# openstack/pyeclib

Measured on AMD Instinct MI355X. Metric: device-resident encode+decode GiB/s, k=10 m=4, 4 MiB objects, 1/2/4/8 GPU, higher is better.
Workload: dtype u16

## Files before the change

### pyeclib_amd/csrc/ec_kernels_impl.hpp

```cpp
#pragma once

#include <algorithm>
#include <cstdlib>
#include <cstddef>
#include <type_traits>
#include <atomic>
#include <map>
#include <mutex>
#include <tuple>
#include <utility>
#include <unordered_map>

#include "crc32.hpp"
#include "crc_device.hpp"
#include "ec_crc.hpp"
#include "ec_kernels.hpp"

namespace ecamd {
namespace {

typedef __attribute__((address_space(3))) char lds_char;
typedef unsigned int v2u __attribute__((ext_vector_type(2)));
typedef unsigned int v4u __attribute__((ext_vector_type(4)));
__device__ __forceinline__ uint2 lds_u64(uint32_t a, uint32_t tab) {
  const v2u v = *reinterpret_cast<const __attribute__((address_space(3))) v2u*>(
      reinterpret_cast<const lds_char*>(static_cast<uintptr_t>(a)) + tab);
  return make_uint2(v.x, v.y);
}
__device__ __forceinline__ uint32_t lds_u32(uint32_t a, uint32_t tab) {
  return *reinterpret_cast<const __attribute__((address_space(3))) uint32_t*>(
      reinterpret_cast<const lds_char*>(static_cast<uintptr_t>(a)) + tab);
}
__device__ __forceinline__ __attribute__((address_space(3))) v4u* lds_v4(uint32_t byte) {
  return reinterpret_cast<__attribute__((address_space(3))) v4u*>(static_cast<uintptr_t>(byte));
}

__device__ __forceinline__ uint4 ld_stream(const void* p) {
  const v4u v = __builtin_nontemporal_load(reinterpret_cast<const v4u*>(p));
  return make_uint4(v.x, v.y, v.z, v.w);
}
__device__ __forceinline__ void st_stream(void* p, const uint4& x) {
  v4u v;
  v.x = x.x;
  v.y = x.y;
  v.z = x.z;
  v.w = x.w;
  __builtin_nontemporal_store(v, reinterpret_cast<v4u*>(p));
}

typedef __amdgpu_buffer_rsrc_t Rsrc;
constexpr int kNt = 2;
__device__ __forceinline__ uint32_t to_sgpr(uint32_t v);
__device__ __forceinline__ Rsrc rsrc(const void* base, int records = -1) {
  const uint64_t a = reinterpret_cast<uint64_t>(base);
  const uint32_t lo = __builtin_amdgcn_readfirstlane(static_cast<uint32_t>(a));
  const uint32_t hi = __builtin_amdgcn_readfirstlane(static_cast<uint32_t>(a >> 32));
  const int n = static_cast<int>(to_sgpr(static_cast<uint32_t>(records)));
  return __builtin_amdgcn_make_buffer_rsrc(
      reinterpret_cast<void*>((static_cast<uint64_t>(hi) << 32) | lo), 0, n, 0x00020000);
}
template <bool CACHED = false>
__device__ __forceinline__ uint4 buf_ld(Rsrc r, uint32_t voff, uint32_t soff) {
  const v4u v = __builtin_amdgcn_raw_buffer_load_b128(r, voff, soff, CACHED ? 0 : kNt);
  return make_uint4(v.x, v.y, v.z, v.w);
}
__device__ __forceinline__ void st_fence() {
  __builtin_amdgcn_sched_barrier(0);
  asm volatile("s_nop 0");
  __builtin_amdgcn_sched_barrier(0);
}

template <bool CACHED = false>
__device__ __forceinline__ void buf_st(Rsrc r, uint32_t voff, uint32_t soff, const uint4& x) {
  v4u v;
  v.x = x.x;
  v.y = x.y;
  v.z = x.z;
  v.w = x.w;
  __builtin_amdgcn_raw_buffer_store_b128(v, r, voff, soff, CACHED ? 0 : kNt);
  st_fence();
}

__device__ __forceinline__ void lookup_fence() {
  __builtin_amdgcn_sched_barrier(0);
  asm volatile("" ::: "memory");
}

__device__ __forceinline__ uint32_t xor3(uint32_t a, uint32_t b, uint32_t c) {
  return __builtin_amdgcn_bitop3_b32(a, b, c, 0x96);
}


#define ECAMD_SDWA_AND_BYTE(B)                                                              \
  "v_and_b32_sdwa %0, %1, %2 dst_sel:DWORD dst_unused:UNUSED_PAD src0_sel:BYTE_" #B \
  " src1_sel:DWORD"
template <int B>
__device__ __forceinline__ uint32_t hi_nib16(uint32_t x) {
// ... 580 lines not shown
__host__ __device__ constexpr int encode_occ() {
  if (F::kRows > kRowsPerPass) return 4;
  if (CRC) return DATA ? kEncodeCrcDataOcc : (stream_bufs<K>() >= 6 ? 6 : kEncodeCrcOcc);
  if (DATA) return kEncodeDataOcc;
  if (NBX > 6) return 4;
  if (F::kW == 8 && K >= 18) return 7;
  return kEncodeOcc;
}

template <class F, int K, int NR, bool NOCOMP = false, bool DATA = false, int CH = 1,
          bool NTL = false, int NBX = 0, bool HEAD = false, bool CRC = false>
__global__ void __launch_bounds__(kThreadsPerBlock)
    __attribute__((amdgpu_waves_per_eu(encode_occ<F, K, DATA, NBX, CRC>(), 8)))
    encode_kernel(EncodeParams p) {
  load_tables(p.tables, K * F::kTableBytes, 0);
  if constexpr (CRC)
    load_tables(static_cast<const uint32_t*>(p.crc_lanes), kCrcLaneBytes, crc_lds_base<F, K>());
  __syncthreads();
  if (p.fused_edges) {
    if (p.edge_blocks == 0) {
      encode_edges<F, K, NR, DATA>(p, gridDim.x - 1 - blockIdx.x, gridDim.x);
    } else if (blockIdx.x < p.edge_blocks) {
      encode_edges<F, K, NR, DATA>(p, blockIdx.x, p.edge_blocks);
      return;
    }
  }
  encode_interior<F, K, NR, NOCOMP, DATA, CH, NTL, NBX, HEAD, CRC>(p);
}

template <class F, int K, int NR>
__global__ void __launch_bounds__(kThreadsPerBlock) encode_edge_kernel(EncodeParams p) {
  load_tables(p.tables, K * F::kTableBytes, 0);
  __syncthreads();
  encode_edges<F, K, NR, false>(p, blockIdx.x, gridDim.x);
}

constexpr uint32_t kDmaSlot = 8192;
constexpr uint32_t kDmaThreads = 512;

typedef unsigned int v4u_s __attribute__((ext_vector_type(4)));
__device__ __forceinline__ v4u_s rsrc4(const void* base, uint32_t records) {
  const uint64_t a = reinterpret_cast<uint64_t>(base);
  v4u_s r;
  r.x = __builtin_amdgcn_readfirstlane(static_cast<uint32_t>(a));
  r.y = __builtin_amdgcn_readfirstlane(static_cast<uint32_t>(a >> 32)) & 0xFFFFu;
  r.z = to_sgpr(records);
  r.w = 0x00020000u;
  return r;
}
template <bool NT>
__device__ __forceinline__ void dma16(v4u_s r, uint32_t voff, uint32_t soff, uint32_t lds) {
  uint32_t keep;
  if constexpr (NT)
    asm volatile(
        "s_mov_b32 %0, m0\n\ts_mov_b32 m0, %3\n\ts_nop 0\n\t"
        "buffer_load_dwordx4 %1, %2, %4 offen nt lds\n\ts_mov_b32 m0, %0"
        : "=&s"(keep) : "v"(voff), "s"(r), "s"(lds), "s"(soff) : "memory");
  else
    asm volatile(
        "s_mov_b32 %0, m0\n\ts_mov_b32 m0, %3\n\ts_nop 0\n\t"
        "buffer_load_dwordx4 %1, %2, %4 offen lds\n\ts_mov_b32 m0, %0"
        : "=&s"(keep) : "v"(voff), "s"(r), "s"(lds), "s"(soff) : "memory");
}
template <int N>
__device__ __forceinline__ void wait_vm() {
  static_assert(N >= 0 && N <= 63, "vmcnt range");
  asm volatile("s_waitcnt vmcnt(%0)" ::"n"(N) : "memory");
}
__device__ __forceinline__ void ring_barrier() {
  asm volatile("s_waitcnt lgkmcnt(0)" ::: "memory");
  __builtin_amdgcn_s_barrier();
  asm volatile("" ::: "memory");
}

template <class F, int K>
__host__ __device__ constexpr uint32_t dma_ring_base() {
  return (K * F::kTableBytes + 255u) & ~255u;
}
template <class F, int K, int R, int SW, int W = 8>
__host__ __device__ constexpr uint32_t dma_lds_bytes(bool crc = false) {
  return dma_ring_base<F, K>() + (crc ? kCrcLaneBytes : 0u) + R * 1024 * W * SW;
}

template <class F, int K, int NR, int R, bool NT, int L = 4, int SW = 1, int W = 8,
          bool DATA = false, bool NOCOMP = false, bool CONTIG = false, int RUNS = 0, int COMB = 0,
          int CV = 6>
__global__ void __launch_bounds__(W * 64) encode_dma_kernel(EncodeParams p) {
  static_assert(R >= 2 && R <= K + 1, "ring of 2 .. K + 1 slots");
  static_assert(L == 2 || L == 4 || L == 8 || L == 16, "loader waves");
  constexpr uint32_t kSlot = 1024u * W * SW;
  constexpr int kPerLoader = kSlot / 1024 / L;
  const uint32_t wave = wave_in_block();
  if (blockIdx.x < p.edge_blocks) {
    if (threadIdx.x >= kThreadsPerBlock) return;
    for (uint32_t i = threadIdx.x; i < K * F::kTableBytes / 16; i += kThreadsPerBlock)
      lds_v4(0)[i] = reinterpret_cast<const v4u*>(p.tables)[i];
    __syncthreads();
    encode_edges<F, K, NR, DATA>(p, blockIdx.x, p.edge_blocks);
    return;
  }
  const bool crc = p.crc_lanes != nullptr;
  for (uint32_t i = threadIdx.x; i < K * F::kTableBytes / 16; i += W * 64)
    lds_v4(0)[i] = reinterpret_cast<const v4u*>(p.tables)[i];
  if (crc)
    load_tables(static_cast<const uint32_t*>(p.crc_lanes), kCrcLaneBytes, dma_ring_base<F, K>(), W * 64);
  __syncthreads();
  ItemRange rg = item_range(p.n_obj * p.tiles, p.xcd_split, interior_block(p.edge_blocks));
  if constexpr (CONTIG) {
    const uint64_t nall = static_cast<uint64_t>(p.n_obj) * p.tiles;
    const IBlock ib = interior_block(p.edge_blocks);
    rg = {static_cast<uint32_t>(__builtin_amdgcn_readfirstlane(static_cast<uint32_t>(nall * ib.b / ib.g))),
          static_cast<uint32_t>(__builtin_amdgcn_readfirstlane(static_cast<uint32_t>(nall * (ib.b + 1) / ib.g))),
          1u};
  }
  uint32_t n_items = 0;
  const IBlock ibk = interior_block(p.edge_blocks);
  const uint32_t nall = p.n_obj * p.tiles;
  const uint32_t runs_total = RUNS ? (nall + RUNS - 1) / RUNS : 0;
  const uint32_t groups = COMB ? ibk.g / COMB : 1, r0 = COMB ? ibk.b % COMB : 0;
  const uint32_t per_obj = COMB ? (p.tiles > r0 ? (p.tiles - r0 + COMB - 1) / COMB : 0) : 0;
  if constexpr (COMB > 0) {
    const uint32_t g0 = ibk.b / COMB;
    if (per_obj == 0 || g0 >= p.n_obj || ibk.b >= groups * COMB) return;
    n_items = to_sgpr((p.n_obj - g0 + groups - 1) / groups * per_obj);
  } else if constexpr (RUNS > 0) {
    if (ibk.b >= runs_total) return;
    n_items = (runs_total - ibk.b + ibk.g - 1) / ibk.g * RUNS;
    if ((runs_total - 1 - ibk.b) % ibk.g == 0) n_items -= runs_total * RUNS - nall;
    n_items = to_sgpr(n_items);
  } else {
    if (rg.begin >= rg.end) return;
    n_items = to_sgpr((rg.end - rg.begin + rg.step - 1) / rg.step);
  }
  const bool loader = wave < static_cast<uint32_t>(L);
  const uint32_t lane16 = lane_id() * 16, lane4 = lane_id() * 4;
  const uint32_t kRing = to_sgpr(dma_ring_base<F, K>() + (crc ? kCrcLaneBytes : 0u));
  const uint32_t chunks = crc_chunks(p.tiles, p.tile_ch);
  auto item_at = [&](uint32_t i, uint32_t& o, uint32_t& x0) {
    if constexpr (COMB > 0) {
      const uint32_t q = i / per_obj, sidx = i - q * per_obj;
      o = to_sgpr(ibk.b / COMB + q * groups);
      x0 = (r0 + sidx * COMB) * kSlot;
      return;
    }
    const uint32_t w = RUNS ? (ibk.b + ibk.g * (i / (RUNS ? RUNS : 1))) * RUNS + i % (RUNS ? RUNS : 1)
                            : rg.begin + i * rg.step;
    o = to_sgpr(w / p.tiles);
    x0 = (w - o * p.tiles) * kSlot;
  };
  auto issue = [&](uint32_t i, int j, uint32_t ri) {
    if (!loader) return;
    uint32_t o, x0;
    const bool valid = i < n_items;
    item_at(valid ? i : 0, o, x0);
    const v4u_s src = rsrc4(p.objs + static_cast<uint64_t>(o) * p.obj_stride, valid ? ~0u : 0u);
    const uint32_t part = wave * (kSlot / L);
    const uint32_t lds = kRing + ri * kSlot + part;
    const uint32_t soff = to_sgpr(j * p.bs + x0 + part);
#pragma unroll
    for (int c = 0; c < kPerLoader; ++c) dma16<NT>(src, lane16, soff + 1024 * c, lds + 1024 * c);
  };
#pragma unroll
  for (int t = 0; t < R - 1; ++t) issue(t / K, t % K, t);
  uint32_t ring = 0;
  typename F::Acc s[SW];
#pragma unroll
  for (int c = 0; c < SW; ++c) F::zero(s[c]);
  constexpr bool kMf = CV == 4 || CV == 6;
  constexpr bool kMf4 = CV == 6;
  constexpr int kPerRow = kMf ? 9 : 5;
  constexpr int kCrcSteps = kPerRow * NR + (kMf4 ? 1 : 0);
  static_assert(!kMf4 || NR <= 4, "one joint wave XOR");
  uint32_t cfin[kMf4 ? 4 : 1] = {};
  uint4 crow[NR];
  uint32_t cacc[NR];
  uint32_t* cpart = p.crc_part;
  bool cpend = false;
  crcdev::mfma_v4i mb[kMf ? 8 : 1];
  crcdev::mfma_v16i macc = {};
  if constexpr (kMf) {
    if (crc) crcdev::mfma_load_b(p.crc_lanes, lane_id(), mb);
  }
  uint32_t dfin[kMf4 && DATA ? 4 : 1] = {};
  uint4 xprev = {};
  uint32_t* dprev = nullptr;
  bool dpend = false;
  auto data_crc = [&](int c, uint32_t* base) {
    if constexpr (kMf4 && DATA) {
      crcdev::mfma_v16i dacc = {};
#pragma unroll
      for (int d = 0; d < 8; ++d) dacc = crcdev::mfma_plane(xprev, d, mb[d], d == 0 ? crcdev::mfma_v16i{} : dacc);
      dfin[c % 4] = crcdev::mfma_lanes(dacc, dma_ring_base<F, K>() + offsetof(CrcLaneTables, mst), lane4);
      if (c % 4 == 3 || c == K - 1) {
        const int n = c % 4 + 1;
        const uint32_t t = crcdev::wave_xor4(dfin[0], n > 1 ? dfin[1] : 0u, n > 2 ? dfin[2] : 0u,
                                             n > 3 ? dfin[3] : 0u, lane_id());
        if (lane_id() < static_cast<uint32_t>(n)) base[c + 1 - n + lane_id()] = t;
      }
    }
  };
  auto crc_step = [&](int u) {
    if constexpr (kMf4) {
      if (u == kPerRow * NR) {
        const uint32_t t = crcdev::wave_xor4(cfin[0], cfin[1], cfin[2], cfin[3], lane_id());
        if (lane_id() < p.nrows && lane_id() < static_cast<uint32_t>(NR)) cpart[lane_id()] = t;
        return;
      }
      const int q = u / kPerRow, d = u % kPerRow;
      if (d < 8)
        macc = crcdev::mfma_plane(crow[q], d, mb[d], d == 0 ? crcdev::mfma_v16i{} : macc);
      else
        cfin[q] = crcdev::mfma_lanes(macc, dma_ring_base<F, K>() + offsetof(CrcLaneTables, mst), lane4);
      return;
    }
    if constexpr (kMf) {
      const int q = u / kPerRow, d = u % kPerRow;
      if (d < 8) {
        macc = crcdev::mfma_plane(crow[q], d, mb[d], d == 0 ? crcdev::mfma_v16i{} : macc);
      } else if (static_cast<uint32_t>(q) < p.nrows) {
        crc_store(cpart + q, crcdev::mfma_finish(macc, dma_ring_base<F, K>() + offsetof(CrcLaneTables, mst), lane4));
      }
      return;
    }
    const int q = u / kPerRow, d = u % kPerRow;
    if (d < 4) {
      const uint32_t w = d == 0 ? crow[q].x : d == 1 ? crow[q].y : d == 2 ? crow[q].z : crow[q].w;
      cacc[q] ^= crcdev::raw_dword(w, d, dma_ring_base<F, K>());
    } else if (static_cast<uint32_t>(q) < p.nrows) {
      crc_store(cpart + q, crcdev::wave_xor(crcdev::lane_map(
                               cacc[q], dma_ring_base<F, K>() + offsetof(CrcLaneTables, lane), lane4)));
    }
  };
#pragma clang loop unroll(disable)
  for (uint32_t i = 0; i < n_items; ++i) {
    uint32_t o, x0;
    item_at(i, o, x0);
    const Rsrc par = rsrc_parity(p, o);
    Rsrc dat;
    if constexpr (DATA) dat = rsrc_data(p, o);
#pragma unroll
    for (int j = 0; j < K; ++j) {
      if (loader) wait_vm<kPerLoader * (R - 2)>();
      ring_barrier();
      const uint32_t rn = ring == 0 ? R - 1 : ring - 1;
      issue(i + (j + R - 1) / K, (j + R - 1) % K, rn);
#pragma unroll
      for (int c = 0; c < SW; ++c) {
        const v4u xin = *lds_v4(kRing + ring * kSlot + (wave * SW + c) * 1024 + lane16);
        const uint4 x = make_uint4(xin.x, xin.y, xin.z, xin.w);
        if constexpr (NOCOMP) {
          uint32_t* a = reinterpret_cast<uint32_t*>(&s[c]);
          a[0] ^= x.x;
        } else {
          F::template mac<true>(F::kb(0), j * F::kTableBytes, x, s[c]);
        }
        if constexpr (DATA) {
          buf_st(dat, lane16, j * p.frag_stride + kHeaderBytes + x0 + (wave * SW + c) * 1024, x);
          uint32_t* dpart = p.crc_part_data + (static_cast<uint64_t>(o) * chunks + x0 / 1024 + wave * SW + c) * K;
          if constexpr (kMf4 && SW == 1) {
            if (crc) {
              if (j > 0) data_crc(j - 1, dpart);
              else if (dpend) data_crc(K - 1, dprev);
              xprev = x;
              if (j == K - 1) {
                dprev = dpart;
                dpend = true;
              }
            }
          } else if (crc) {
            crc_store(dpart + j, crcdev::chunk_crc(x, dma_ring_base<F, K>(), lane4));
          }
        }
      }
      if constexpr (SW == 1 && (CV == 0 || CV == 4 || CV == 6)) {
        if (cpend) {
#pragma unroll
          for (int u = j * kCrcSteps / K; u < (j + 1) * kCrcSteps / K; ++u) crc_step(u);
        }
      }
      ring = ring + 1 == R ? 0 : ring + 1;
    }
#pragma unroll
    for (int c = 0; c < SW; ++c) {
      F::pin(s[c]);
      const uint32_t soff = p.row0 * p.frag_stride + kHeaderBytes + x0 + (wave * SW + c) * 1024;
#pragma unroll
      for (int q = 0; q < NR; ++q)
        buf_st(parity_row<NR>(p, o, q, par), lane16, soff + q * p.frag_stride, F::row(s[c], q));
      if (crc) {
        uint32_t* part = p.crc_part + (static_cast<uint64_t>(o) * chunks + x0 / 1024 + wave * SW + c) * p.m + p.row0;
        if constexpr (SW == 1 && (CV == 0 || CV == 4 || CV == 6)) {
#pragma unroll
          for (int q = 0; q < NR; ++q) {
            crow[q] = F::row(s[c], q);
            cacc[q] = 0;
          }
          cpart = part;
          cpend = true;
        } else {
#pragma unroll
          for (int q = 0; q < NR; ++q)
            if (static_cast<uint32_t>(q) < p.nrows)
              crc_store(part + q, crcdev::chunk_crc<CV == 2>(F::row(s[c], q), dma_ring_base<F, K>(), lane4));
        }
      }
      F::zero(s[c]);
    }
  }
  if constexpr (kMf4 && DATA && SW == 1) {
    if (crc && dpend) data_crc(K - 1, dprev);
  }
  if constexpr (SW == 1 && (CV == 0 || CV == 4 || CV == 6)) {
    if (cpend) {
#pragma unroll
      for (int u = 0; u < kCrcSteps; ++u) crc_step(u);
    }
  }
  if (loader) wait_vm<0>();
}

__global__ void __launch_bounds__(kThreadsPerBlock) __attribute__((unused))
    copy_data_kernel(EncodeParams p) {
  const uint32_t per_frag = (p.bs + kTile - 1) / kTile;
  const uint32_t per_obj = p.k * per_frag;
  const uint32_t items = p.n_obj * per_obj;
  for (uint32_t w = blockIdx.x; w < items; w += gridDim.x) {
    const uint32_t o = w / per_obj, rest = w - o * per_obj;
    const uint32_t j = rest / per_frag, c = rest - j * per_frag;
    const uint32_t t = c * kTile + threadIdx.x * 16;
    if (t >= p.bs) continue;
    const uint8_t* obj = p.objs + static_cast<uint64_t>(o) * p.obj_stride;
    const uint4 x = load_clamped(obj, static_cast<uint64_t>(j) * p.bs + t, p.obj_len);
    store_partial(p.data + static_cast<uint64_t>(o) * p.stripe_stride + j * p.frag_stride +
                      kHeaderBytes + t,
                  x, static_cast<int64_t>(p.bs) - t);
  }
}


struct Slots {
  uint32_t table;
  uint32_t slot;
};

template <class F, int K>
struct TablePre {
  static constexpr int kChunks = K * F::kTableBytes / 16;
  static constexpr int kPer = (kChunks + kThreadsPerBlock - 1) / kThreadsPerBlock;
  uint4 v[kPer];
  uint32_t table;
};

template <class F, int K>
__device__ __forceinline__ void table_prefetch(const DecodeParams& p, uint32_t table, bool need,
                                               TablePre<F, K>& pre) {
  constexpr uint32_t kBytes = K * F::kTableBytes;
  const Rsrc t = rsrc(p.tables + static_cast<uint64_t>(table) * (kBytes / 4), need ? kBytes : 0);
#pragma unroll
  for (int i = 0; i < TablePre<F, K>::kPer; ++i)
    pre.v[i] = buf_ld<true>(t, (threadIdx.x + i * kThreadsPerBlock) * 16, 0);
  pre.table = need ? table : 0xFFFFFFFFu;
}

template <class F, int K, class D>
__device__ __forceinline__ uint32_t ensure_tables(const DecodeParams& p, const D& d, Slots& st,
                                                  const TablePre<F, K>& pre) {
  constexpr uint32_t kSlot = table_slot_bytes(K, F::kW);
  if (d.n_out() != 0 && d.table() != st.table) {
    st.slot ^= 1u;
    const uint32_t base = st.slot * kSlot;
    if (pre.table == d.table()) {
      auto* dst = lds_v4(base);
#pragma unroll
      for (int i = 0; i < TablePre<F, K>::kPer; ++i) {
        const uint32_t c = threadIdx.x + i * kThreadsPerBlock;
        if (c < static_cast<uint32_t>(TablePre<F, K>::kChunks)) {
          v4u v;
          v.x = pre.v[i].x;
          v.y = pre.v[i].y;
          v.z = pre.v[i].z;
          v.w = pre.v[i].w;
          dst[c] = v;
        }
      }
    } else {
      load_tables(p.tables + static_cast<uint64_t>(d.table()) * (K * F::kTableBytes / 4),
                  K * F::kTableBytes, base, kThreadsPerBlock);
    }
    __syncthreads();
// ... 563 lines not shown
  hipEvent_t fork = nullptr, join = nullptr;
};

template <class Main, class Side>
hipError_t fork_join(hipStream_t stream, Main main, Side side) {
  static std::mutex mu;
  static SideStream per_dev[64];
  std::lock_guard<std::mutex> lk(mu);
  int dev = 0;
  SideStream* sd = nullptr;
  if (ab_knob("ECAMD_EDGE_SIDE", 0) == 2) {
    const hipError_t e = side(stream);
    return e != hipSuccess ? e : main(stream);
  }
  if (hipGetDevice(&dev) == hipSuccess && dev >= 0 && dev < 64) {
    sd = &per_dev[dev];
    if (sd->s == nullptr &&
        (hipStreamCreateWithFlags(&sd->s, hipStreamNonBlocking) != hipSuccess ||
         hipEventCreateWithFlags(&sd->fork, hipEventDisableTiming) != hipSuccess ||
         hipEventCreateWithFlags(&sd->join, hipEventDisableTiming) != hipSuccess)) {
      (void)hipGetLastError();
      sd->s = nullptr;
      sd = nullptr;
    }
  }
  if (sd == nullptr) {
    const hipError_t e = side(stream);
    return e != hipSuccess ? e : main(stream);
  }
  hipError_t e = hipEventRecord(sd->fork, stream);
  if (e == hipSuccess) e = hipStreamWaitEvent(sd->s, sd->fork, 0);
  if (e != hipSuccess) return e;
  const hipError_t em = main(stream);
  const hipError_t es = side(sd->s);
  e = hipEventRecord(sd->join, sd->s);
  if (e == hipSuccess) e = hipStreamWaitEvent(stream, sd->join, 0);
  return em != hipSuccess ? em : (es != hipSuccess ? es : e);
}

inline int64_t last_room(uint32_t bs, uint64_t obj_len, uint32_t k) {
  int64_t room = static_cast<int64_t>(obj_len) - static_cast<int64_t>(k - 1) * bs;
  if (room > static_cast<int64_t>(bs)) room = bs;
  return room < 0 ? 0 : room;
}

inline void set_tiles(EncodeParams& p, int64_t room, uint32_t ch) {
  p.tile_ch = ch;
  p.tiles = static_cast<uint32_t>(room / (kTile * ch));
  p.edge_tiles = (p.bs + kTile - 1) / kTile - p.tiles * ch;
}

inline hipError_t crc_finish(uint8_t* frags, uint64_t frag_stride, uint64_t stripe_stride,
                             const uint32_t* part, uint32_t part_rows, uint32_t part_row0,
                             const void* lanes, const void* tables, uint32_t n_obj, uint32_t count,
                             uint32_t bs, uint32_t chunks, hipStream_t stream) {
  CrcFinishParams fp{};
  fp.frags = frags;
  fp.frag_stride = frag_stride;
  fp.stripe_stride = stripe_stride;
  fp.part = part;
  fp.part_rows = part_rows;
  fp.part_row0 = part_row0;
  fp.lanes = lanes;
  fp.tables = tables;
  fp.n_obj = n_obj;
  fp.count = count;
  fp.bs = bs;
  fp.chunks = chunks;
  return launch_crc_finish(fp, stream);
}

template <int K>
hipError_t encode_crc_finish(const EncodeParams& p, bool data, uint32_t chunks, hipStream_t stream) {
  hipError_t e = crc_finish(p.parity + static_cast<uint64_t>(p.row0) * p.frag_stride, p.frag_stride,
                            p.stripe_stride, p.crc_part, p.m, p.row0, p.crc_lanes,
                            p.crc_finish_tables, p.n_obj, p.nrows, p.bs, chunks, stream);
  if (e != hipSuccess || !data) return e;
  return crc_finish(p.data, p.frag_stride, p.stripe_stride, p.crc_part_data, K, 0, p.crc_lanes,
                    p.crc_finish_tables, p.n_obj, K, p.bs, chunks, stream);
}

template <class F, int K, int NR, int R, bool NT, int L = 4, int SW = 1, int W = 8,
          bool DATA = false, bool NOCOMP = false, bool CONTIG = false, int RUNS = 0, int COMB = 0,
          int CV = 6>
hipError_t launch_encode_dma(EncodeParams p, hipStream_t stream, uint32_t* chunks = nullptr,
                             bool xcd = true) {
  set_tiles(p, last_room(p.bs, p.obj_len, K), 1024u * W * SW / kTile);
  if (chunks) *chunks = crc_chunks(p.tiles, p.tile_ch);
  const auto kern = encode_dma_kernel<F, K, NR, R, NT, L, SW, W, DATA, NOCOMP, CONTIG, RUNS, COMB, CV>;
  const size_t lds = dma_lds_bytes<F, K, R, SW, W>(p.crc_lanes != nullptr);
  if (!lds_starts_at_zero(reinterpret_cast<const void*>(kern))) return hipErrorInvalidKernelFile;
  const int cus = device_cus();
  const uint32_t items = p.n_obj * p.tiles;
  const uint32_t edge_items = std::max(p.n_obj * p.edge_tiles, p.headers ? p.n_obj : 0u);
  const uint32_t e = (std::min<uint32_t>(edge_items, static_cast<uint32_t>(cus)) + 7u) & ~7u;
  uint32_t g = std::min<uint32_t>(static_cast<uint32_t>(cus) & ~7u, std::max(items, 1u));
  if (g >= 8) g &= ~7u;
  p.edge_blocks = edge_items ? e : 0;
  p.fused_edges = 1;
  p.xcd_split = xcd_split_for(static_cast<int>(g), xcd);
  hipLaunchKernelGGL(kern, dim3(g + p.edge_blocks), dim3(W * 64), lds, stream, p);
  return hipGetLastError();
}

template <class F, int K, int NR>
hipError_t launch_encode_ab(EncodeParams p, hipStream_t stream, bool data, uint32_t edge_items) {
  constexpr size_t lds = K * F::kTableBytes;
  const int per_cu = ab_knob("ECAMD_ENC_PER_CU", kEncodePerCu);
  if (p.crc_lanes != nullptr) return hipErrorNotSupported;
  if (ab_knob("ECAMD_EDGE_SIDE", 0)) {
    p.fused_edges = 0;
    hipError_t e = fork_join(
        stream,
        [&](hipStream_t s) { return launch(encode_kernel<F, K, NR>, p, lds, p.n_obj * p.tiles, s, per_cu); },
        [&](hipStream_t s) {
          return launch(encode_edge_kernel<F, K, NR>, p, lds,
                        std::max(p.n_obj * p.edge_tiles, p.headers ? p.n_obj : 0u), s);
        });
    if (e != hipSuccess || !data) return e;
    return launch(copy_data_kernel, p, 0, p.n_obj * K * ((p.bs + kTile - 1) / kTile), stream);
  }
  p.fused_edges = 1;
  const uint32_t items = p.n_obj * p.tiles;
  if (data && ab_knob("ECAMD_DATA_COPY", 0)) {
    const hipError_t e = launch_edges_apart(encode_kernel<F, K, NR>, p, lds, items, edge_items,
                                            stream, per_cu, true);
    if (e != hipSuccess) return e;
    return launch(copy_data_kernel, p, 0, p.n_obj * K * ((p.bs + kTile - 1) / kTile), stream);
  }
  if constexpr (K == 10 && NR == 4) {
    const bool ntl = ab_knob("ECAMD_ENC_NTL", 0);
    if (!data) {
      const int ring = ab_knob("ECAMD_ENC_DMA", 0);
      const int lw = ab_knob("ECAMD_ENC_DMA_L", 4), sw = ab_knob("ECAMD_ENC_DMA_SW", 1);
      const int nw = ab_knob("ECAMD_ENC_DMA_W", 8);
      if (ring == 5 && lw == 4 && sw == 1 && nw == 8) return launch_encode_dma<F, K, NR, 5, true>(p, stream);
      if (ring == 3 && lw == 4 && sw == 2 && nw == 8) return launch_encode_dma<F, K, NR, 3, true, 4, 2>(p, stream);
      if (ring == 3 && lw == 8 && sw == 2 && nw == 8) return launch_encode_dma<F, K, NR, 3, true, 8, 2>(p, stream);
      if (ring == 2 && lw == 4 && sw == 4 && nw == 8) return launch_encode_dma<F, K, NR, 2, true, 4, 4>(p, stream);
      if (ring == 3 && lw == 4 && sw == 4 && nw == 8) return launch_encode_dma<F, K, NR, 3, true, 4, 4>(p, stream);
      if (ring == 3 && lw == 4 && sw == 1 && nw == 16) return launch_encode_dma<F, K, NR, 3, true, 4, 1, 16>(p, stream);
      if (ring == 3 && lw == 8 && sw == 1 && nw == 16) return launch_encode_dma<F, K, NR, 3, true, 8, 1, 16>(p, stream);
      if (ring == 4 && lw == 4 && sw == 1 && nw == 16) return launch_encode_dma<F, K, NR, 4, true, 4, 1, 16>(p, stream);
      if (ring == 3 && lw == 4 && sw == 2 && nw == 16) return launch_encode_dma<F, K, NR, 3, true, 4, 2, 16>(p, stream);
      if (ring == 3 && lw == 2 && sw == 1 && nw == 16) return launch_encode_dma<F, K, NR, 3, true, 2, 1, 16>(p, stream);
      if (ring == 3 && lw == 4 && sw == 1 && nw == 12) return launch_encode_dma<F, K, NR, 3, true, 4, 1, 12>(p, stream);
      if (ring == 4 && lw == 4 && sw == 1 && nw == 12) return launch_encode_dma<F, K, NR, 4, true, 4, 1, 12>(p, stream);
      if (ring == 4 && lw == 4 && sw == 1 && nw == 8) return launch_encode_dma<F, K, NR, 4, true, 4, 1, 8>(p, stream);
      if (ring == 5 && lw == 4 && sw == 1 && nw == 12) return launch_encode_dma<F, K, NR, 5, true, 4, 1, 12>(p, stream);
      if (ring == -3 && lw == 4 && sw == 1 && nw == 16) return launch_encode_dma<F, K, NR, 3, false, 4, 1, 16>(p, stream);
      if (ab_knob("ECAMD_ENC_DMA_NOCOMP", 0))
        return launch_encode_dma<F, K, NR, 3, true, 4, 1, 12, false, true>(p, stream);
      if (ab_knob("ECAMD_ENC_DMA_CONTIG", 0) == 12)
        return launch_encode_dma<F, K, NR, 3, true, 4, 1, 12, false, false, true>(p, stream);
      if (ab_knob("ECAMD_ENC_DMA_CONTIG", 0) == 16)
        return launch_encode_dma<F, K, NR, 3, true, 4, 1, 16, false, false, true>(p, stream);
      const int runs = ab_knob("ECAMD_ENC_DMA_RUNS", 0);
      if (runs == 2) return launch_encode_dma<F, K, NR, 3, true, 4, 1, 16, false, false, false, 2>(p, stream);
      if (runs == 4) return launch_encode_dma<F, K, NR, 3, true, 4, 1, 16, false, false, false, 4>(p, stream);
      if (runs == 8) return launch_encode_dma<F, K, NR, 3, true, 4, 1, 16, false, false, false, 8>(p, stream);
      const int comb = ab_knob("ECAMD_ENC_DMA_COMB", 0);
      if (comb == 4) return launch_encode_dma<F, K, NR, 3, true, 4, 1, 16, false, false, false, 0, 4>(p, stream);
      if (comb == 5) return launch_encode_dma<F, K, NR, 3, true, 4, 1, 16, false, false, false, 0, 5>(p, stream);
      if (comb == 8) return launch_encode_dma<F, K, NR, 3, true, 4, 1, 16, false, false, false, 0, 8>(p, stream);
      if (comb == 16) return launch_encode_dma<F, K, NR, 3, true, 4, 1, 16, false, false, false, 0, 16>(p, stream);
    }
    if (ab_knob("ECAMD_ENC_NOCOMP", 0))
      return ntl ? launch_edges_apart(encode_kernel<F, K, NR, true, false, 1, true>, p, lds, items,
                                      edge_items, stream, per_cu, true)
                 : launch_edges_apart(encode_kernel<F, K, NR, true>, p, lds, items, edge_items,
                                      stream, per_cu, true);
    if (!data && ab_knob("ECAMD_ENC_R3", 0))
      return launch_edges_apart(encode_kernel<F, K, NR, false, false, 1, false, 0, false>, p, lds,
                                items, edge_items, stream, per_cu, true);
  }
  if (per_cu != kEncodePerCu)
    return data ? launch_edges_apart(encode_kernel<F, K, NR, false, true>, p, lds, items,
                                     edge_items, stream, per_cu, true)
                : launch_edges_apart(encode_kernel<F, K, NR>, p, lds, items, edge_items, stream,
                                     per_cu, true);
  return hipErrorNotSupported;
}

template <class F, int K, int NR>
hipError_t launch_encode_k(EncodeParams p, hipStream_t stream) {
  const int64_t room = last_room(p.bs, p.obj_len, K);
  set_tiles(p, room, 1);
  constexpr size_t lds = K * F::kTableBytes;
  const bool data = p.data != nullptr && p.row0 == 0;
  const uint32_t edge_items = std::max(p.n_obj * p.edge_tiles, p.headers ? p.n_obj : 0u);
  if constexpr (kAB && F::kRows <= kRowsPerPass) {
    const hipError_t e = launch_encode_ab<F, K, NR>(p, stream, data, edge_items);
    if (e != hipErrorNotSupported) return e;
  }
  if constexpr (kAB && F::kRows > kRowsPerPass) {
    const int per_cu = ab_knob("ECAMD_ENC_PER_CU", kEncode8PerCu);
    if (per_cu != kEncode8PerCu && !data && p.crc_lanes == nullptr) {
      p.fused_edges = 1;
      return launch_edges_apart(encode_kernel<F, K, NR>, p, lds, p.n_obj * p.tiles, edge_items,
                                stream, per_cu, true);
    }
  }
  const bool crc = p.crc_lanes != nullptr;
  uint32_t chunks = 0;
  hipError_t e = hipErrorInvalidValue;
  bool done = false;
  if constexpr (kAB && K == 10 && NR == 4) {
    const int cv = ab_knob("ECAMD_CRC_V", 0), cr = ab_knob("ECAMD_CRC_R", 3);
    if (!crc && ab_knob("ECAMD_ENC_CV0", 0))
      return data ? launch_encode_dma<F, K, NR, 4, true, 4, 1, 8, true, false, false, 0, 0, 0>(p, stream, &chunks, false)
                  : launch_encode_dma<F, K, NR, 3, true, 4, 1, 12, false, false, false, 0, 0, 0>(p, stream, &chunks);
    if (crc && data && cv == 10) {
      e = launch_encode_dma<F, K, NR, 4, true, 4, 1, 8, true, false, false, 0, 0, 0>(p, stream, &chunks, false);
      if (e != hipSuccess) return e;
      return encode_crc_finish<K>(p, data, chunks, stream);
    }
    if (crc && !data && (cv != 0 || cr != 3)) {
      if (cv == 10 && cr == 3) e = launch_encode_dma<F, K, NR, 3, true, 4, 1, 12, false, false, false, 0, 0, 0>(p, stream, &chunks);
      else if (cv == 1 && cr == 3) e = launch_encode_dma<F, K, NR, 3, true, 4, 1, 12, false, false, false, 0, 0, 1>(p, stream, &chunks);
      else if (cv == 2 && cr == 3) e = launch_encode_dma<F, K, NR, 3, true, 4, 1, 12, false, false, false, 0, 0, 2>(p, stream, &chunks);
      else if (cv == 10 && cr == 4) e = launch_encode_dma<F, K, NR, 4, true, 4, 1, 12, false, false, false, 0, 0, 0>(p, stream, &chunks);
      else if (cv == 1 && cr == 4) e = launch_encode_dma<F, K, NR, 4, true, 4, 1, 12, false, false, false, 0, 0, 1>(p, stream, &chunks);
      else if (cv == 4 && cr == 3) e = launch_encode_dma<F, K, NR, 3, true, 4, 1, 12, false, false, false, 0, 0, 4>(p, stream, &chunks);
      else if (cv == 4 && cr == 4) e = launch_encode_dma<F, K, NR, 4, true, 4, 1, 12, false, false, false, 0, 0, 4>(p, stream, &chunks);
      else return hipErrorInvalidValue;
      if (e != hipSuccess) return e;
      return encode_crc_finish<K>(p, data, chunks, stream);
    }
  }
  if constexpr (F::kRows <= kRowsPerPass && K >= kDmaMinK) {
    if (crc || data ||
        ((NR > 2 || !ab_knob("ECAMD_ENC_STREAM2", 0)) &&
         dma_batch(K, p.bs, p.obj_len, p.n_obj, device_cus(), p.direct) && !ab_knob("ECAMD_ENC_STREAM", 0))) {
      if (static_cast<uint64_t>(K) * p.bs + 65536u > 0xFFFFFFFFull) return hipErrorInvalidValue;
      if constexpr (kAB && K == 10 && NR == 4) {
        const int dw = ab_knob("ECAMD_ENC_DATA_W", 8), dr = ab_knob("ECAMD_ENC_DATA_R", 4);
        if (data && (dw != 8 || dr != 4)) {
          if (dw == 16 && dr == 3) e = launch_encode_dma<F, K, NR, 3, true, 4, 1, 16, true>(p, stream, &chunks);
          else if (dw == 12 && dr == 4) e = launch_encode_dma<F, K, NR, 4, true, 4, 1, 12, true>(p, stream, &chunks);
          else if (dw == 12 && dr == 3) e = launch_encode_dma<F, K, NR, 3, true, 4, 1, 12, true>(p, stream, &chunks);
          else if (dw == 8 && dr == 3) e = launch_encode_dma<F, K, NR, 3, true, 4, 1, 8, true>(p, stream, &chunks);
          else if (dw == 8 && dr == 5) e = launch_encode_dma<F, K, NR, 5, true, 4, 1, 8, true>(p, stream, &chunks);
          else return hipErrorInvalidValue;
          if (e != hipSuccess || !crc) return e;
          return encode_crc_finish<K>(p, data, chunks, stream);
        }
      }
      if constexpr (std::is_same_v<F, Gf16<2>> && NR == 4) {
        if (data && crc) {
          e = launch_encode_dma<F, K, NR, 3, true, 4, 1, 12, true>(p, stream, &chunks);
          return e != hipSuccess ? e : encode_crc_finish<K>(p, data, chunks, stream);
        }
      }
      e = data ? launch_encode_dma<F, K, NR, 4, true, 4, 1, 8, true>(p, stream, &chunks, false)
               : launch_encode_dma<F, K, NR, 3, true, 4, 1, 12>(p, stream, &chunks);
      done = true;
    }
  }
  if (!done) {
    p.fused_edges = 1;
    const uint32_t items = p.n_obj * p.tiles;
    chunks = crc_chunks(p.tiles, p.tile_ch);
    if constexpr (F::kRows > kRowsPerPass) {
      if (crc) return hipErrorInvalidValue;
      e = data ? launch_edges_apart(encode_kernel<F, K, NR, false, true>, p, lds, items, edge_items,
                                    stream, kEncodePerCu, true)
               : launch_edges_apart(encode_kernel<F, K, NR>, p, lds, items, edge_items, stream,
                                    kEncode8PerCu, true);
    } else if constexpr (K < kDmaMinK) {
      const size_t crc_lds = crc_lds_base<F, K>() + kCrcLaneBytes;
      if (crc)
        e = data ? launch_edges_apart(encode_kernel<F, K, NR, false, true, 1, false, 0, false, true>, p,
                                      crc_lds, items, edge_items, stream, kEncodePerCu, true)
                 : launch_edges_apart(encode_kernel<F, K, NR, false, false, 1, false, 0, false, true>, p,
                                      crc_lds, items, edge_items, stream, kEncodePerCu, true);
      else
        e = data ? launch_edges_apart(encode_kernel<F, K, NR, false, true>, p, lds, items, edge_items,
                                      stream, kEncodePerCu, true)
                 : launch_edges_apart(encode_kernel<F, K, NR>, p, lds, items, edge_items, stream,
                                      kEncodePerCu, true);
    } else {
      e = launch_edges_apart(encode_kernel<F, K, NR>, p, lds, items, edge_items, stream,
                             kEncodePerCu, true);
    }
  }
  if (e != hipSuccess || !crc) return e;
  return encode_crc_finish<K>(p, data, chunks, stream);
}

template <class F, int K>
constexpr uint32_t decode_lds_bytes() {
  return 2 * table_slot_bytes(K, F::kW);
}

template <class F, int K, int R, bool NT, int L = 4, int W = 16, int PROBE = 0, int PER_CU = 1,
          int MODE = kDecode>
hipError_t launch_decode_dma(DecodeParams p, hipStream_t stream) {
  p.tile_ch = W / 4;
  const int64_t lim = MODE == kReconstruct ? static_cast<int64_t>(p.bs) : last_room(p.bs, p.obj_len, K);
  p.tiles = static_cast<uint32_t>(lim / (1024 * W));
  p.edge_tiles = (p.bs + kTile - 1) / kTile - p.tiles * p.tile_ch;
  const auto kern = decode_dma_kernel<F, K, R, NT, L, W, PROBE, MODE>;
  constexpr size_t lds = 2 * table_slot_bytes(K, F::kW) + R * 1024 * W;
  if (!lds_starts_at_zero(reinterpret_cast<const void*>(kern))) return hipErrorInvalidKernelFile;
  const int cus = device_cus();
  const uint32_t items = p.n_obj * p.tiles;
  const uint32_t edge_items =
      std::max(p.n_obj * p.edge_tiles, MODE == kReconstruct && p.headers ? p.n_obj : 0u);
  const uint32_t e = (std::min<uint32_t>(edge_items, static_cast<uint32_t>(cus)) + 7u) & ~7u;
  uint32_t g = std::min<uint32_t>((static_cast<uint32_t>(cus) * PER_CU) & ~7u, std::max(items, 1u));
  if (g >= 8) g &= ~7u;
  p.edge_blocks = edge_items ? e : 0;
  p.fused_edges = 1;
  p.xcd_split = xcd_split_for(static_cast<int>(g), kDecodeXcd);
  hipLaunchKernelGGL(kern, dim3(g + p.edge_blocks), dim3(W * 64), lds, stream, p);
  return hipGetLastError();
}
// ... 110 lines not shown
```

Before: 3075.

## Defer parity row stores and spread them across next item's ring steps

Instead of storing all NR parity rows at the end of each item, the encode DMA kernel keeps the previous item's parity rows in registers and issues one row store at evenly spaced slots during the next item's K-step loop. The loader vmcnt waits are adjusted per step to count the interleaved stores, and dummy stores are added in the prologue so the counter arithmetic stays uniform. The aim is to smooth the store burst and overlap parity writes with loads and compute. An AT_END knob keeps the old behaviour. The cost is extra live registers and more complex waitcnt logic.

New measurement: 3105, median of 6. Within noise of the previous version (+1.0%).

```diff
diff --git a/pyeclib_amd/csrc/dma_wait.hpp b/pyeclib_amd/csrc/dma_wait.hpp
--- /dev/null
+++ b/pyeclib_amd/csrc/dma_wait.hpp
@@ -0,0 +1,23 @@
+#pragma once
+
+namespace dmawait {
+
+constexpr int row_slot(int q, int K, int NR) { return ((2 * q + 1) * K) / (2 * NR); }
+
+constexpr int rows_in_slot(int j, int K, int NR) {
+  int n = 0;
+  for (int q = 0; q < NR; ++q) n += row_slot(q, K, NR) == j ? 1 : 0;
+  return n;
+}
+
+constexpr int wait_base(int R, int kPer, int S) { return S + (R - 2) * (kPer + S); }
+constexpr int rows_before(int j, int K, int R, int NR) {
+  int n = 0;
+  for (int d = 1; d <= R - 1; ++d) n += rows_in_slot(j - d < 0 ? j - d + K : j - d, K, NR);
+  return n;
+}
+constexpr int loader_wait(int j, int K, int R, int kPer, int NR, int S) {
+  return wait_base(R, kPer, S) + rows_before(j, K, R, NR);
+}
+
+}
diff --git a/pyeclib_amd/csrc/ec_kernels_impl.hpp b/pyeclib_amd/csrc/ec_kernels_impl.hpp
--- a/pyeclib_amd/csrc/ec_kernels_impl.hpp
+++ b/pyeclib_amd/csrc/ec_kernels_impl.hpp
@@ -13,6 +13,7 @@
 
 #include "crc32.hpp"
 #include "crc_device.hpp"
+#include "dma_wait.hpp"
 #include "ec_crc.hpp"
 #include "ec_kernels.hpp"
 
@@ -759,14 +760,33 @@
   return dma_ring_base<F, K>() + (crc ? kCrcLaneBytes : 0u) + R * 1024 * W * SW;
 }
 
+constexpr int kDeferMaxK = 16;
+template <int BASE, int MAXR, int I = 0>
+__device__ __forceinline__ void wait_vm_plus(int r) {
+  if constexpr (I < MAXR) {
+    if (r == I)
+      wait_vm<BASE + I>();
+    else
+      wait_vm_plus<BASE, MAXR, I + 1>(r);
+  } else {
+    wait_vm<BASE + MAXR>();
+  }
+}
+template <int K, int R, int PER, int NR, int S>
+__device__ __forceinline__ void loader_wait(int j) {
+  wait_vm_plus<dmawait::wait_base(R, PER, S), NR>(dmawait::rows_before(j, K, R, NR));
+}
+
 template <class F, int K, int NR, int R, bool NT, int L = 4, int SW = 1, int W = 8,
           bool DATA = false, bool NOCOMP = false, bool CONTIG = false, int RUNS = 0, int COMB = 0,
-          int CV = 6>
+          int CV = 6, bool AT_END = false>
 __global__ void __launch_bounds__(W * 64) encode_dma_kernel(EncodeParams p) {
   static_assert(R >= 2 && R <= K + 1, "ring of 2 .. K + 1 slots");
   static_assert(L == 2 || L == 4 || L == 8 || L == 16, "loader waves");
   constexpr uint32_t kSlot = 1024u * W * SW;
   constexpr int kPerLoader = kSlot / 1024 / L;
+  constexpr bool kDefer = SW == 1 && !AT_END && !DATA && NR == 4 && K <= kDeferMaxK;
+  constexpr int kS = DATA ? 1 : 0;
   const uint32_t wave = wave_in_block();
   if (blockIdx.x < p.edge_blocks) {
     if (threadIdx.x >= kThreadsPerBlock) return;
@@ -838,8 +858,21 @@
     for (int c = 0; c < kPerLoader; ++c) dma16<NT>(src, lane16, soff + 1024 * c, lds + 1024 * c);
   };
 #pragma unroll
-  for (int t = 0; t < R - 1; ++t) issue(t / K, t % K, t);
+  for (int t = 0; t < R - 1; ++t) {
+    issue(t / K, t % K, t);
+    if constexpr (kDefer) {
+      if (loader) {
+        const Rsrc none = rsrc(p.parity, 0);
+        if constexpr (DATA) buf_st(none, lane16, 0, make_uint4(0, 0, 0, 0));
+#pragma unroll
+        for (int q = 0; q < NR; ++q)
+          if (dmawait::row_slot(q, K, NR) == (t - (R - 1) + K) % K) buf_st(none, lane16, 0, make_uint4(0, 0, 0, 0));
+      }
+    }
+  }
   uint32_t ring = 0;
+  uint32_t po = 0, px0 = 0;
+  bool ppend = false;
   typename F::Acc s[SW];
 #pragma unroll
   for (int c = 0; c < SW; ++c) F::zero(s[c]);
@@ -912,12 +945,20 @@
   for (uint32_t i = 0; i < n_items; ++i) {
     uint32_t o, x0;
     item_at(i, o, x0);
-    const Rsrc par = rsrc_parity(p, o);
+    [[maybe_unused]] const Rsrc par = rsrc_parity(p, o);
     Rsrc dat;
     if constexpr (DATA) dat = rsrc_data(p, o);
+    [[maybe_unused]] const Rsrc ppar = rsrc(p.parity + static_cast<uint64_t>(po) * p.stripe_stride,
+                           ppend ? static_cast<int>(p.m * static_cast<uint32_t>(p.frag_stride)) : 0);
+    [[maybe_unused]] const uint32_t psoff = p.row0 * p.frag_stride + kHeaderBytes + px0 + wave * 1024;
 #pragma unroll
     for (int j = 0; j < K; ++j) {
-      if (loader) wait_vm<kPerLoader * (R - 2)>();
+      if (loader) {
+        if constexpr (kDefer)
+          loader_wait<K, R, kPerLoader, NR, kS>(j);
+        else
+          wait_vm<kPerLoader * (R - 2)>();
+      }
       ring_barrier();
       const uint32_t rn = ring == 0 ? R - 1 : ring - 1;
       issue(i + (j + R - 1) / K, (j + R - 1) % K, rn);
@@ -955,15 +996,29 @@
           for (int u = j * kCrcSteps / K; u < (j + 1) * kCrcSteps / K; ++u) crc_step(u);
         }
       }
+      if constexpr (kDefer) {
+#pragma unroll
+        for (int q = 0; q < NR; ++q)
+          if (dmawait::row_slot(q, K, NR) == j)
+            buf_st(parity_row<NR>(p, po, q, ppar), lane16, psoff + q * p.frag_stride, crow[q]);
+      }
       ring = ring + 1 == R ? 0 : ring + 1;
     }
 #pragma unroll
     for (int c = 0; c < SW; ++c) {
       F::pin(s[c]);
-      const uint32_t soff = p.row0 * p.frag_stride + kHeaderBytes + x0 + (wave * SW + c) * 1024;
-#pragma unroll
-      for (int q = 0; q < NR; ++q)
-        buf_st(parity_row<NR>(p, o, q, par), lane16, soff + q * p.frag_stride, F::row(s[c], q));
+      [[maybe_unused]] const uint32_t soff = p.row0 * p.frag_stride + kHeaderBytes + x0 + (wave * SW + c) * 1024;
+      if constexpr (kDefer) {
+#pragma unroll
+        for (int q = 0; q < NR; ++q) crow[q] = F::row(s[c], q);
+        po = o;
+        px0 = x0;
+        ppend = true;
+      } else {
+#pragma unroll
+        for (int q = 0; q < NR; ++q)
+          buf_st(parity_row<NR>(p, o, q, par), lane16, soff + q * p.frag_stride, F::row(s[c], q));
+      }
       if (crc) {
         uint32_t* part = p.crc_part + (static_cast<uint64_t>(o) * chunks + x0 / 1024 + wave * SW + c) * p.m + p.row0;
         if constexpr (SW == 1 && (CV == 0 || CV == 4 || CV == 6)) {
@@ -982,6 +1037,15 @@
         }
       }
       F::zero(s[c]);
+    }
+  }
+  if constexpr (kDefer) {
+    if (ppend) {
+      const Rsrc ppar = rsrc_parity(p, po);
+      const uint32_t psoff = p.row0 * p.frag_stride + kHeaderBytes + px0 + wave * 1024;
+#pragma unroll
+      for (int q = 0; q < NR; ++q)
+        buf_st(parity_row<NR>(p, po, q, ppar), lane16, psoff + q * p.frag_stride, crow[q]);
     }
   }
   if constexpr (kMf4 && DATA && SW == 1) {
@@ -1711,12 +1775,12 @@
 
 template <class F, int K, int NR, int R, bool NT, int L = 4, int SW = 1, int W = 8,
           bool DATA = false, bool NOCOMP = false, bool CONTIG = false, int RUNS = 0, int COMB = 0,
-          int CV = 6>
+          int CV = 6, bool AT_END = false>
 hipError_t launch_encode_dma(EncodeParams p, hipStream_t stream, uint32_t* chunks = nullptr,
                              bool xcd = true) {
   set_tiles(p, last_room(p.bs, p.obj_len, K), 1024u * W * SW / kTile);
   if (chunks) *chunks = crc_chunks(p.tiles, p.tile_ch);
-  const auto kern = encode_dma_kernel<F, K, NR, R, NT, L, SW, W, DATA, NOCOMP, CONTIG, RUNS, COMB, CV>;
+  const auto kern = encode_dma_kernel<F, K, NR, R, NT, L, SW, W, DATA, NOCOMP, CONTIG, RUNS, COMB, CV, AT_END>;
   const size_t lds = dma_lds_bytes<F, K, R, SW, W>(p.crc_lanes != nullptr);
   if (!lds_starts_at_zero(reinterpret_cast<const void*>(kern))) return hipErrorInvalidKernelFile;
   const int cus = device_cus();
@@ -1862,6 +1926,20 @@
         ((NR > 2 || !ab_knob("ECAMD_ENC_STREAM2", 0)) &&
          dma_batch(K, p.bs, p.obj_len, p.n_obj, device_cus(), p.direct) && !ab_knob("ECAMD_ENC_STREAM", 0))) {
       if (static_cast<uint64_t>(K) * p.bs + 65536u > 0xFFFFFFFFull) return hipErrorInvalidValue;
+      if constexpr (kAB && !std::is_same_v<F, Gf8> && (K == 10 || K == 12)) {
+        if (ab_knob("ECAMD_ROWS_AT_END", 0)) {
+          if constexpr (NR == 4) {
+            if (data && crc) {
+              e = launch_encode_dma<F, K, NR, 3, true, 4, 1, 12, true, false, false, 0, 0, 6, true>(p, stream, &chunks);
+              return e != hipSuccess ? e : encode_crc_finish<K>(p, data, chunks, stream);
+            }
+          }
+          e = data ? launch_encode_dma<F, K, NR, 4, true, 4, 1, 8, true, false, false, 0, 0, 6, true>(p, stream, &chunks, false)
+                   : launch_encode_dma<F, K, NR, 3, true, 4, 1, 12, false, false, false, 0, 0, 6, true>(p, stream, &chunks);
+          if (e != hipSuccess || !crc) return e;
+          return encode_crc_finish<K>(p, data, chunks, stream);
+        }
+      }
       if constexpr (kAB && K == 10 && NR == 4) {
         const int dw = ab_knob("ECAMD_ENC_DATA_W", 8), dr = ab_knob("ECAMD_ENC_DATA_R", 4);
         if (data && (dw != 8 || dr != 4)) {
```
